# 12334zq/optical-flow-1

Hardware: AMD Instinct MI355X
Metric: Mpix*warp-iters/s, TV-L1 1920x1080 5-scale (higher is better)
Workload: dtype f64; 1 GPU; tvl1flow 1920x1080 pair (synthetic P1), nscales=5 warps=5 tau=0.25 lambda=0.15 theta=0.3 zfactor=0.5 epsilon=0.01; one pair per step per GPU; workload_name=1080p, arithmetic_mode=tolerance, pairs_per_gpu=1040, pairs_in_flight_per_gpu=64, lockstep_group=16, streams_per_gpu=4, distinct_pairs=8

## Files before the change

optical-flow-1_amd/csrc/ofx_tvl1.hip:

```cpp
#include "ofx_ops.h"
#include "ofx_device.h"
#include "ofx_loop.h"

#include <atomic>
#include <chrono>
#include <cmath>
#include <thread>
#include <type_traits>

#define TVL1_GRAD_IS_ZERO 1E-10
#define TVL1_PRESMOOTHING_SIGMA 0.8
#define STRIP_OUT 62

template <typename T> OFX_DEV double rnd_to(double x);
template <> OFX_DEV double rnd_to<double>(double x) { return x; }
template <> OFX_DEV double rnd_to<float>(double x) { return (double) (float) x; }

#ifdef OFX_NO_RFL
#define OFX_WAVE_UNIFORM(x) (x)
#else
#define OFX_WAVE_UNIFORM(x) __builtin_amdgcn_readfirstlane(x)
#endif
template <typename T> struct RowIn {
    double2 u, p1, p2, a;
// ... 753 lines not shown
    const bool idle = (strip >= strips_x) || (y0 >= ny);
    const int yend = (y0 + rows < ny) ? y0 + rows : ny;
    const int ys = y0 > N - 1 ? y0 - (N - 1) : 0;
    const int yl = (yend + N - 1 < ny - 1) ? yend + N - 1 : ny - 1;
    const int c = strip * STRIP3_OUT - STRIP3_HALO + lane;
    const int cc = c < 0 ? 0 : (c > nx - 1 ? nx - 1 : c);
    const bool lef = (c == 0), rig = (c == nx - 1);
    const bool owner = (lane >= STRIP3_HALO) && (lane < STRIP3_OUT + STRIP3_HALO) && (c < nx);
    const unsigned E2 = 2 * sizeof(T);
    const unsigned row2 = (unsigned) nx * E2;
    const unsigned off = ((unsigned) ys * nx + cc) * E2;
    const unsigned so = ((unsigned) ys * nx + (c < 0 ? 0 : c)) * E2;
    double up12 = 0.0, up22 = 0.0;
    RowIn<T> cur;
    if (!idle) {
        if (ys > 0) {
            up12 = ldw2(at(P1in, off - row2)).y;
            up22 = ldw2(at(P2in, off - row2)).y;
        }
        cur = tvl1_load_row<T>(Uin, P1in, P2in, A, R, off);
    }
    if (check) {
        double e1 = 0.0;
#pragma unroll
        for (int i = 0; i < N; i++) {
            if (k0 - i > 0) {
                const double e = loop_error_from_sum(wave_allreduce_sum(prev[i]), nx * ny, OFX_CRIT_MEAN);
                if (!(e > eps2)) return;
                if (i == 0) e1 = e;
            }
        }
        if (dev) {
            niter = (k0 > 0 && e1 <= eps2 * afac1) ? 1 : ((k0 > 0 && e1 <= eps2 * afac2) ? 2 : 3);
            if (N == 4 && niter == 3 && !(k0 > 0 && e1 <= eps2 * afac3)) niter = 4;
            if (niter > max_iter - k0) niter = max_iter - k0;
            if (scribe) dev->cursor[(launch + 1) & 1][g] = k0 + niter;
        }
    }
    if (idle) return;
    const int step = check ? 1 : 0;
    if (N == 4 && niter >= 4) {
        if constexpr (N == 4)
            tvl1_iter3_march<T, NT, STRICT, 4, N>(Uin, P1in, P2in, A, R, hu.out, h1.out, h2.out, err, slot0, step, gw, nx, ny, y0, yend,
                                                  ys, yl, lef, rig, owner, off, so, up12, up22, cur, l_t, theta, taut, ring);
    } else if (niter >= 3)
        tvl1_iter3_march<T, NT, STRICT, 3, N>(Uin, P1in, P2in, A, R, hu.out, h1.out, h2.out, err, slot0, step, gw, nx, ny, y0, yend, ys,
                                              yl, lef, rig, owner, off, so, up12, up22, cur, l_t, theta, taut);
    else if (niter == 2)
        tvl1_iter3_march<T, NT, STRICT, 2, N>(Uin, P1in, P2in, A, R, hu.out, h1.out, h2.out, err, slot0, step, gw, nx, ny, y0, yend, ys,
                                              yl, lef, rig, owner, off, so, up12, up22, cur, l_t, theta, taut);
    else
        tvl1_iter3_march<T, NT, STRICT, 1, N>(Uin, P1in, P2in, A, R, hu.out, h1.out, h2.out, err, slot0, step, gw, nx, ny, y0, yend, ys,
                                              yl, lef, rig, owner, off, so, up12, up22, cur, l_t, theta, taut);
}

template <typename T, bool NT, bool STRICT>
__global__ __launch_bounds__(256) __attribute__((amdgpu_waves_per_eu(OFX_ITER3_WAVES, OFX_ITER3_WAVES))) void k_tvl1_iter3(
    Tri<typename Pix<T>::v2> Ut, Tri<typename Pix<T>::v2> P1t, Tri<typename Pix<T>::v2> P2t,
    const typename Pix<T>::v2 *__restrict__ Ag, const T *__restrict__ Rg, double *__restrict__ errg, int k0, int check, int slot0,
    int nx, int ny, int rows, int strips_x, int strips_pad, double l_t, double theta, double taut, double eps2, unsigned incode,
    unsigned runmask, unsigned long long nit, int err_stride, OfxLoopDev *dev, int launch, double afac1, double afac2, double afac3,
    int max_iter)
{
    tvl1_unit<T, NT, STRICT, 3>(Ut, P1t, P2t, Ag, Rg, errg, k0, check, slot0, nx, ny, rows, strips_x, strips_pad, l_t, theta, taut, eps2,
                                incode, runmask, nit, err_stride, dev, launch, afac1, afac2, afac3, max_iter, nullptr);
}

template <typename T, bool NT, bool STRICT>
__global__ __launch_bounds__(256) __attribute__((amdgpu_waves_per_eu(OFX_ITER3_WAVES, OFX_ITER3_WAVES))) void k_tvl1_iter4(
    Tri<typename Pix<T>::v2> Ut, Tri<typename Pix<T>::v2> P1t, Tri<typename Pix<T>::v2> P2t,
    const typename Pix<T>::v2 *__restrict__ Ag, const T *__restrict__ Rg, double *__restrict__ errg, int k0, int check, int slot0,
    int nx, int ny, int rows, int strips_x, int strips_pad, double l_t, double theta, double taut, double eps2, unsigned incode,
    unsigned runmask, unsigned long long nit, int err_stride, OfxLoopDev *dev, int launch, double afac1, double afac2, double afac3,
    int max_iter)
{
    __shared__ Tvl1Ring rings[4];
    tvl1_unit<T, NT, STRICT, 4>(Ut, P1t, P2t, Ag, Rg, errg, k0, check, slot0, nx, ny, rows, strips_x, strips_pad, l_t, theta, taut, eps2,
                                incode, runmask, nit, err_stride, dev, launch, afac1, afac2, afac3, max_iter, &rings[threadIdx.x >> 6]);
}

#define TILE_RH 16
template <typename T, bool STRICT, int K>
__global__ __launch_bounds__(64 * TILE_RH) void k_tvl1_tile(
    Tri<typename Pix<T>::v2> Ut, Tri<typename Pix<T>::v2> P1t, Tri<typename Pix<T>::v2> P2t,
    const typename Pix<T>::v2 *__restrict__ Ag, const T *__restrict__ Rg, double *__restrict__ errg, int k0, int check, int slot0,
    int nx, int ny, int tiles_x, double l_t, double theta, double taut, double eps2, unsigned incode, unsigned runmask,
    unsigned long long nit, int err_stride)
{
    using v2 = typename Pix<T>::v2;
    static_assert(K < 16, "4 bits of `nit` per pair");
    __shared__ double2 s_p[2][TILE_RH][64];
    __shared__ double2 s_u[2][TILE_RH][64];
    const int lane = threadIdx.x & 63, w = threadIdx.x >> 6;
    const int g = blockIdx.y;
    if (!((runmask >> g) & 1u)) return;
    const int niter = (int) ((nit >> (4 * g)) & 15ull);
    const size_t npix = (size_t) nx * ny;
    const TriSel<v2> hu = pick3(Ut, incode, g, npix), h1 = pick3(P1t, incode, g, npix), h2 = pick3(P2t, incode, g, npix);
    double *__restrict__ err = errg + (size_t) g * err_stride;
    double prev[K];
#pragma unroll
    for (int i = 0; i < K; i++) prev[i] = (check && k0 - i > 0) ? loop_fetch_prev(err, k0 - i) : 0.0;

    constexpr int OW = 64 - 2 * K, OH = TILE_RH - 2 * K;
    const int tx = blockIdx.x % tiles_x, ty = blockIdx.x / tiles_x;
    const int c = tx * OW - K + lane, y = ty * OH - K + w;
    const int cc = c < 0 ? 0 : (c > nx - 1 ? nx - 1 : c), yc = y < 0 ? 0 : (y > ny - 1 ? ny - 1 : y);
    const bool inside = (c >= 0) && (c < nx) && (y >= 0) && (y < ny);
    const bool owner = inside && lane >= K && lane < 64 - K && w >= K && w < TILE_RH - K;
    const bool lef = (c == 0), rig = (c == nx - 1), top = (y == 0), bot = (y == ny - 1);
    const size_t p = (size_t) yc * nx + cc;
    double2 u = ldw2(hu.in + p), p1 = ldw2(h1.in + p), p2 = ldw2(h2.in + p);
    const double2 a = ldw2(Ag + (size_t) g * npix + p);
    const double r = ldw(Rg + (size_t) g * npix + p);
    if (check) {
#pragma unroll
        for (int i = 0; i < K; i++)
            if (k0 - i > 0 && !(loop_error_from_sum(wave_allreduce_sum(prev[i]), nx * ny, OFX_CRIT_MEAN) > eps2)) return;
    }
    double acc[K];
#pragma unroll
    for (int it = 0; it < K; it++) {
        acc[it] = 0.0;
        if (it < niter) {
            s_p[it & 1][w][lane] = make_double2(p1.y, p2.y);
            __syncthreads();
            const double2 up = s_p[it & 1][w > 0 ? w - 1 : 0][lane];
            const double l11 = wave_shift_up(p1.x), l21 = wave_shift_up(p2.x);
            const double2 un = tvl1_primal<T, STRICT>(u, a, r, p1, p2, l11, l21, up.x, up.y, lef, rig, top, bot, l_t, theta);
            if (owner) acc[it] = TVL1_TOL64<T, STRICT> ? du2_fma(un, u)
                : (un.x - u.x) * (un.x - u.x) + (un.y - u.y) * (un.y - u.y);
            s_u[it & 1][w][lane] = un;
            __syncthreads();
            const double2 dn = s_u[it & 1][w < TILE_RH - 1 ? w + 1 : w][lane];
            const double r1 = wave_shift_down(un.x), r2 = wave_shift_down(un.y);
            double2 q1, q2;
            tvl1_dual<T, STRICT>(p1, p2, un, r1, r2, dn, rig, bot, taut, q1, q2);
            u = un;
            p1 = make_double2(rnd_to<T>(q1.x), rnd_to<T>(q1.y));
            p2 = make_double2(rnd_to<T>(q2.x), rnd_to<T>(q2.y));
        }
    }
    if (owner) {
        const size_t po = (size_t) y * nx + c;
        stn2(hu.out + po, u);
        stn2(h1.out + po, p1);
        stn2(h2.out + po, p2);
    }
#pragma unroll
    for (int it = 0; it < K; it++)
        if (it < niter) loop_accumulate(err, slot0 + (check ? it : 0), acc[it], blockIdx.x * TILE_RH + w);
}

#ifndef OFX_WARP_BX
#define OFX_WARP_BX 64
#define OFX_WARP_BY 4
#endif
template <typename T>
__global__ void k_tvl1_warp(const typename Pix<T>::v2 *__restrict__ pag, const T *__restrict__ pbg, const T *__restrict__ I0g,
                            Tri<typename Pix<T>::v2> Ut,
                            typename Pix<T>::v2 *__restrict__ Ag, T *__restrict__ Rg, int nx, int ny, unsigned curcode)
{
    const int j = blockIdx.x * OFX_WARP_BX + threadIdx.x;
    const int i = blockIdx.y * OFX_WARP_BY + threadIdx.y;
    if (j >= nx || i >= ny) return;
    const int g = blockIdx.z;
    const size_t goff = (size_t) g * nx * ny;
    const typename Pix<T>::v2 *__restrict__ pa = pag + goff;
    const T *__restrict__ pb = pbg + goff;
    const T *__restrict__ I0 = I0g + goff;
    const typename Pix<T>::v2 *__restrict__ U = pick3(Ut, curcode, g, (size_t) nx * ny).in;
    typename Pix<T>::v2 *__restrict__ A = Ag + goff;
    T *__restrict__ R = Rg + goff;
    const size_t p = (size_t) i * nx + j;
    const double2 u = ldw2(U + p);
    const BicubicTaps t = bicubic_taps(j + u.x, i + u.y, nx, ny);
    double I1w = 0.0, I1wx = 0.0, I1wy = 0.0;
    if (!t.out) {
        bicubic_sample3(pa, pb, t, nx, I1w, I1wx, I1wy);
        I1wx = rnd_to<T>(I1wx);
        I1wy = rnd_to<T>(I1wy);
    }
    stn2(A + p, make_double2(I1wx, I1wy));
    stn(R + p, (I1w - I1wx * u.x - I1wy * u.y - ldw(I0 + p)));
}

#ifndef WARP_TW
#define WARP_TW 48
#define WARP_TH 16
#endif
#ifndef WARP_BY
#define WARP_BY 8
#endif
#ifndef WARP_WAVES
#define WARP_WAVES 8
#endif
#define WARP_ATTR __attribute__((amdgpu_waves_per_eu(WARP_WAVES, WARP_WAVES)))
#define WARP_NT (32 * WARP_BY)
#define WARP_NW (WARP_NT / 64)
template <typename T>
__global__ __launch_bounds__(WARP_NT) WARP_ATTR void k_tvl1_warp_lds(
    const typename Pix<T>::v2 *__restrict__ pag, const T *__restrict__ pbg, const T *__restrict__ I0g,
    Tri<typename Pix<T>::v2> Ut, typename Pix<T>::v2 *__restrict__ Ag, T *__restrict__ Rg, int nx, int ny,
    unsigned curcode)
{
    __shared__ double2 s_a[WARP_TH * WARP_TW];
    __shared__ double s_b[WARP_TH * WARP_TW];
    __shared__ int s_box[WARP_NW][4];
    const int tid = threadIdx.y * 32 + threadIdx.x, wave = tid >> 6;
    const int j = blockIdx.x * 32 + threadIdx.x;
    const int i = blockIdx.y * WARP_BY + threadIdx.y;
    const bool inside = (j < nx) && (i < ny);
    const int g = blockIdx.z;
    const size_t goff = (size_t) g * nx * ny;
    const typename Pix<T>::v2 *__restrict__ pa = pag + goff;
    const T *__restrict__ pb = pbg + goff;
    const typename Pix<T>::v2 *__restrict__ U = pick3(Ut, curcode, g, (size_t) nx * ny).in;
    const size_t p = (size_t) (inside ? i : 0) * nx + (inside ? j : 0);
    double2 u = make_double2(0.0, 0.0);
    BicubicTaps t;
    t.out = true;
    if (inside) {
        u = ldw2(U + p);
        t = bicubic_taps(j + u.x, i + u.y, nx, ny);
    }
    const bool need = inside && !t.out;
    int xlo = need ? t.col[0] : 0x7fffffff, xhi = need ? t.col[3] : -1;
    int ylo = need ? t.row[0] : 0x7fffffff, yhi = need ? t.row[3] : -1;
#pragma unroll
    for (int m = 32; m >= 1; m >>= 1) {
        xlo = min(xlo, __shfl_xor(xlo, m, 64)); xhi = max(xhi, __shfl_xor(xhi, m, 64));
        ylo = min(ylo, __shfl_xor(ylo, m, 64)); yhi = max(yhi, __shfl_xor(yhi, m, 64));
    }
    if ((tid & 63) == 0) { s_box[wave][0] = xlo; s_box[wave][1] = xhi; s_box[wave][2] = ylo; s_box[wave][3] = yhi; }
    __syncthreads();
#pragma unroll
    for (int w = 0; w < WARP_NW; w++) {
        xlo = min(xlo, s_box[w][0]); xhi = max(xhi, s_box[w][1]);
        ylo = min(ylo, s_box[w][2]); yhi = max(yhi, s_box[w][3]);
    }
    const int W = xhi - xlo + 1, H = yhi - ylo + 1;
    const bool any = (xhi >= 0);
    const bool tile = any && W <= WARP_TW && H <= WARP_TH;
    if (tile) {
        for (int k = tid; k < W * H; k += WARP_NT) {
            const int r = k / W, c = k - r * W;
            const size_t src = (size_t) (ylo + r) * nx + (xlo + c);
            s_a[r * WARP_TW + c] = ldw2(pa + src);
            s_b[r * WARP_TW + c] = ldw(pb + src);
        }
        __syncthreads();
    }
    if (!inside) return;
    double I1w = 0.0, I1wx = 0.0, I1wy = 0.0;
    if (need) {
        if (tile) {
            const int cx = t.col[0] - xlo, cy = t.row[0] - ylo;
            double c0[4], c1[4], c2[4];
#pragma unroll
            for (int k = 0; k < 4; k++) {
                const int o = cy * WARP_TW + cx + k;
                const double2 a0 = s_a[o], a1 = s_a[o + WARP_TW], a2 = s_a[o + 2 * WARP_TW], a3 = s_a[o + 3 * WARP_TW];
                const double b0 = s_b[o], b1 = s_b[o + WARP_TW], b2 = s_b[o + 2 * WARP_TW], b3 = s_b[o + 3 * WARP_TW];
                c0[k] = cubic_cell(a0.x, a1.x, a2.x, a3.x, t.fy);
                c1[k] = cubic_cell(a0.y, a1.y, a2.y, a3.y, t.fy);
                c2[k] = cubic_cell(b0, b1, b2, b3, t.fy);
            }
            I1w = cubic_cell(c0[0], c0[1], c0[2], c0[3], t.fx);
            I1wx = cubic_cell(c1[0], c1[1], c1[2], c1[3], t.fx);
            I1wy = cubic_cell(c2[0], c2[1], c2[2], c2[3], t.fx);
        } else {
            bicubic_sample3(pa, pb, t, nx, I1w, I1wx, I1wy);
        }
        I1wx = rnd_to<T>(I1wx);
        I1wy = rnd_to<T>(I1wy);
    }
    stn2(Ag + goff + p, make_double2(I1wx, I1wy));
    stn(Rg + goff + p, (I1w - I1wx * u.x - I1wy * u.y - ldw(I0g + goff + p)));
}

template <typename T>
__global__ void k_tvl1_zoom_in_g(Tri<typename Pix<T>::v2> Ut, unsigned curcode, typename Pix<T>::v2 *__restrict__ Uout, int nx,
                                 int ny, int nxx, int nyy, double fx, double fy, double scale)
{
    const int j1 = blockIdx.x * 64 + threadIdx.x;
    const int i1 = blockIdx.y * 4 + threadIdx.y;
    if (j1 >= nxx || i1 >= nyy) return;
    const int g = blockIdx.z;
    const typename Pix<T>::v2 *__restrict__ U = pick3(Ut, curcode, g, (size_t) nx * ny).in;
    const double i2 = i1 / fy, j2 = j1 / fx;
    const BicubicTaps t = bicubic_taps(j2, i2, nx, ny);
    double c1[4], c2[4];
#pragma unroll
    for (int k = 0; k < 4; k++) {
        const double2 v0 = ldw2(U + (size_t) t.row[0] * nx + t.col[k]);
        const double2 v1 = ldw2(U + (size_t) t.row[1] * nx + t.col[k]);
        const double2 v2 = ldw2(U + (size_t) t.row[2] * nx + t.col[k]);
        const double2 v3 = ldw2(U + (size_t) t.row[3] * nx + t.col[k]);
        c1[k] = cubic_cell(v0.x, v1.x, v2.x, v3.x, t.fy);
        c2[k] = cubic_cell(v0.y, v1.y, v2.y, v3.y, t.fy);
    }
    double2 r;
    r.x = cubic_cell(c1[0], c1[1], c1[2], c1[3], t.fx) * scale;
    r.y = cubic_cell(c2[0], c2[1], c2[2], c2[3], t.fx) * scale;
    stn2(Uout + (size_t) g * nxx * nyy + (size_t) i1 * nxx + j1, r);
}

template <typename T>
__global__ void k_tvl1_to_flo_g(Tri<typename Pix<T>::v2> Ut, unsigned curcode, OfxGroupPtrs out, size_t n)
{
    const size_t i = (size_t) blockIdx.x * blockDim.x + threadIdx.x;
    if (i >= n) return;
    const int g = blockIdx.y;
    const double2 v = ldw2(pick3(Ut, curcode, g, n).in + i);
    ((float2 *) out.a[g])[i] = make_float2((float) v.x, (float) v.y);
}

template <typename T> struct Tvl1Level {
    using v2 = typename Pix<T>::v2;
    using v4 = typename Pix<T>::v4;
    int nx, ny, G;
    int shared;
    T  *I0, *I1;
    v2 *pa;
    T  *pb;
    v2 *U[3], *P1[3], *P2[3], *A;
    T  *R;
    unsigned cur;
    int last_n[OFX_MAX_GROUP];
    size_t n() const { return (size_t) nx * ny; }
    unsigned curidx(int g) const { return (cur >> (2 * g)) & 3u; }
    v2 *Ucur(int g) const { return U[curidx(g)] + (size_t) g * n(); }
    v2 *P1cur(int g) const { return P1[curidx(g)] + (size_t) g * n(); }
    v2 *P2cur(int g) const { return P2[curidx(g)] + (size_t) g * n(); }
    Tri<v2> Ut() const { return Tri<v2>{U[0], U[1], U[2]}; }
    Tri<v2> P1t() const { return Tri<v2>{P1[0], P1[1], P1[2]}; }
    Tri<v2> P2t() const { return Tri<v2>{P2[0], P2[1], P2[2]}; }
};

struct Tvl1Params {
    double tau, lambda, theta, epsilon;
    int warps, verbose, max_iter;
    bool fixed;
};

template <typename T> static int tvl1_level_alloc(ofx_ctx *ctx, Tvl1Level<T> &L, int nx, int ny, int G, bool images, int shared = 0)
{
    const size_t n = (size_t) nx * ny * G;
    L.nx = nx;
    L.ny = ny;
    L.G = G;
    L.shared = shared;
    L.cur = 0;
    for (int g = 0; g < OFX_MAX_GROUP; g++) L.last_n[g] = 0;
    L.I0 = L.I1 = nullptr;
    if (images) {
        OFX_TRY(ofx_alloc(ctx, n, &L.I0));
        if (!shared) OFX_TRY(ofx_alloc(ctx, n, &L.I1));
    }
    OFX_TRY(ofx_alloc(ctx, n, &L.pa));
    OFX_TRY(ofx_alloc(ctx, n, &L.pb));
    for (int h = 0; h < 3; h++) {
        OFX_TRY(ofx_alloc(ctx, n, &L.U[h]));
        OFX_TRY(ofx_alloc(ctx, n, &L.P1[h]));
        OFX_TRY(ofx_alloc(ctx, n, &L.P2[h]));
    }
    OFX_TRY(ofx_alloc(ctx, n, &L.A));
    OFX_TRY(ofx_alloc(ctx, n, &L.R));
    return OFX_OK;
}

static int tvl1_pick_rows(const ofx_ctx *ctx, int nx, int ny, int G)
{
    if (ctx->rows_per_wave > 0) return ctx->rows_per_wave;
    const long strips = (long) ofx_cdiv(nx, STRIP_OUT) * G;
    if (strips * ofx_cdiv(ny, 4) >= 2048) return 4;
    if (strips * ofx_cdiv(ny, 2) >= 1024) return 2;
    return 1;
}

static int tvl1_pick_rows2(const ofx_ctx *ctx, int nx, int ny, int G)
{
    if (ctx->rows_per_wave2 > 0) return ctx->rows_per_wave2;
    const long strips_pad = (long) ofx_cdiv(ofx_cdiv(nx, STRIP2_OUT), 4) * 4 * G;
    const int rmax = 24;
    int best = rmax;
    long best_cost = -1;
    if (ctx->concurrency > 1) {
        static const int cand[] = {1, 2, 3, 4, 5, 6, 8, 10, 12, 14, 16, 20, 24};
        for (int r : cand) {
            const long waves = strips_pad * ofx_cdiv(ny, r);
            const long slots = ctx->rows_slots > 0 ? ctx->rows_slots : 1024;
            const long cost = ((waves + slots - 1) / slots) * (r + 5);
            if (best_cost < 0 || cost < best_cost) { best_cost = cost; best = r; }
        }
        return best;
    }
    const long slots = 1024L * OFX_ITER2_WAVES;
    for (int k = 1; k <= 4; k++) {
        for (int r = 1; r <= rmax; r++) {
            if (strips_pad * ofx_cdiv(ny, r) > k * slots) continue;
            const long cost = (long) k * (r + 5);
            if (best_cost < 0 || cost < best_cost) { best_cost = cost; best = r; }
            break;
        }
    }
    if (best < 3 && strips_pad * ofx_cdiv(ny, 3) >= 512) best = 3;
    return best;
}

static int tvl1_pick_chunk(const ofx_ctx *ctx, int nx, int ny, int G)
{
    if (ctx->chunk > 0) return ctx->chunk;
    const double est_us = fmax(5.0, (double) nx * ny * G * 120.0 / 4.0e6);
    int c = (int) (40.0 / est_us);
    return c < 4 ? 4 : (c > 50 ? 50 : c);
}

static int tvl1_pick_tile(const ofx_ctx *ctx, int nx, int ny, int G)
{
    if (!ctx->tile || !ctx->fuse2) return 0;
    const double lim = ctx->tile_max_px > 0 ? ctx->tile_max_px : 200000.0;
    if ((double) nx * ny * G > lim) return 0;
    return ctx->tile == 6 ? 6 : 4;
}

template <typename T> struct Tvl1Level;
struct Tvl1Params;
template <typename T>
static int tvl1_run_iterations_tile(ofx_ctx *ctx, Tvl1Level<T> &L, const Tvl1Params &P, LoopSpec S, int K, int *n_out,
                                    double *err_out, float *ms_out, int *alt_out);
template <typename T>
static int tvl1_run_iterations_tri(ofx_ctx *ctx, Tvl1Level<T> &L, const Tvl1Params &P, LoopSpec S, int N, int *n_out, double *err_out,
                                   float *ms_out, int *alt_out);

static int tvl1_pick_rows3(const ofx_ctx *ctx, int nx, int ny, int G, int N = 3)
{
    const int depth = 2 * N + 1;
    if (ctx->rows_per_wave3 > 0) return ctx->rows_per_wave3;
    {
        static const char *tab = getenv("OFX_ROWS3");
        for (const char *q = tab; q && *q;) {
            int lny = 0, r = 0;
            if (sscanf(q, "%d:%d", &lny, &r) == 2 && lny == ny && r > 0) return r;
            q = strchr(q, '/');
            if (q) q++;
        }
    }
    const long strips_pad = (long) ofx_cdiv(ofx_cdiv(nx, STRIP3_OUT), 4) * 4 * G;
    const int rmax = 32;
    int best = rmax;
    long best_cost = -1;
    if (ctx->concurrency > 1) {
        static const int cand[] = {2, 3, 4, 5, 6, 8, 10, 12, 14, 16, 20, 24, 28, 32, 36, 40, 48, 54, 64, 72, 80, 96};
        for (int r : cand) {
            if (r > ctx->rows3_max) break;
            const long waves = strips_pad * ofx_cdiv(ny, r);
            const long slots = ctx->rows_slots > 0 ? ctx->rows_slots : 1024;
            const long cost = ((waves + slots - 1) / slots) * (r + depth);
            if (best_cost < 0 || cost < best_cost) { best_cost = cost; best = r; }
        }
        return best;
    }
    const long slots = 1024L * OFX_ITER3_WAVES;
    for (int k = 1; k <= 4; k++) {
        for (int r = 1; r <= rmax; r++) {
            if (strips_pad * ofx_cdiv(ny, r) > k * slots) continue;
            const long cost = (long) k * (r + depth);
            if (best_cost < 0 || cost < best_cost) { best_cost = cost; best = r; }
            break;
        }
    }
    if (best < 4 && strips_pad * ofx_cdiv(ny, 4) >= 512) best = 4;
    return best;
}

#ifndef TVL1_FUSE4_AUTO_PX
#define TVL1_FUSE4_AUTO_PX 2e6
#endif
template <typename T>
static int tvl1_run_iterations(ofx_ctx *ctx, Tvl1Level<T> &L, const Tvl1Params &P, int *n_out, double *err_out,
                               float *ms_out, int *alt_out = nullptr,
                               int *unit_out = nullptr)
{
    const int nx = L.nx, ny = L.ny, G = L.G;
    if ((long long) nx * ny >= (1LL << 27)) return ofx_fail(ctx, OFX_ERR_ARG, "tvl1: image larger than 2^27 pixels");
    const double l_t = P.lambda * P.theta, taut = P.tau / P.theta, theta = P.theta;
    const bool pairs = ctx->fuse2 != 0;
    const int rows = tvl1_pick_rows(ctx, nx, ny, G);
    const int strips_x = ofx_cdiv(nx, STRIP_OUT), strips_pad = ofx_cdiv(strips_x, 4) * 4;
    const unsigned gx1 = (unsigned) (strips_pad / 4) * ofx_cdiv(ny, rows);
    const dim3 block(256);
    const int rows2 = tvl1_pick_rows2(ctx, nx, ny, G);
    const int strips2_x = ofx_cdiv(nx, STRIP2_OUT), strips2_pad = ofx_cdiv(strips2_x, 4) * 4;
    const dim3 grid2((unsigned) (strips2_pad / 4) * ofx_cdiv(ny, rows2), G);
    LoopSpec S;
    S.max_iter = P.max_iter;
    S.size = nx * ny;
    S.thr = P.epsilon * P.epsilon;
    S.crit = OFX_CRIT_MEAN;
    S.chunk = tvl1_pick_chunk(ctx, nx, ny, G);
    S.fixed = P.fixed;
    S.pairs = pairs;
    const int tileK = tvl1_pick_tile(ctx, nx, ny, G);
    if (unit_out) *unit_out = tileK ? tileK : (pairs ? 2 : 1);
    if (tileK) return tvl1_run_iterations_tile<T>(ctx, L, P, S, tileK, n_out, err_out, ms_out, alt_out);
    {
        const bool strict_mode = sizeof(T) == sizeof(double) && !ctx->relaxed_dual;
        const double px = (double) nx * ny * G;
        const bool tri = ctx->fuse3 == 1 ? px >= ctx->fuse3_min_px
                                         : (ctx->fuse3 == 2 && !strict_mode && (G >= 2 || ctx->concurrency > 1) &&
                                            px >= (ctx->fuse3_min_px > 0 ? ctx->fuse3_min_px : 5e5));
        const bool quad = ctx->fuse4 == 1 ? px >= ctx->fuse4_min_px
                                          : (ctx->fuse4 == 2 && tri && ctx->fuse3 == 2 &&
// ... 81 lines not shown
    S.afac = 0.0;
    if (ctx->chunk <= 0) S.chunk = 6 * K;
    const int err_stride = (S.max_iter + 1) * OFX_NSHARD;
    const unsigned all = (G >= 32) ? 0xFFFFFFFFu : ((1u << G) - 1u);
    unsigned b0[OFX_MAX_GROUP];
    for (int g = 0; g < G; g++) b0[g] = L.curidx(g);
    auto go = [&](int k0, int check, int slot0, double thr, unsigned incode, unsigned runmask, unsigned long long nit) -> int {
        auto kern = K == 6 ? k_tvl1_tile<T, false, 6> : k_tvl1_tile<T, false, 4>;
        if constexpr (sizeof(T) == sizeof(double)) {
            if (strict) kern = K == 6 ? k_tvl1_tile<T, true, 6> : k_tvl1_tile<T, true, 4>;
        }
        hipLaunchKernelGGL(kern, grid, block, 0, ctx->stream, L.Ut(), L.P1t(), L.P2t(), L.A, (const T *) L.R, ctx->d_err, k0, check,
                           slot0, nx, ny, tiles_x, l_t, theta, taut, thr, incode, runmask, nit, err_stride);
        OFX_LAUNCH_CHECK(ctx);
        return OFX_OK;
    };
    auto launch = [&](int k, int cnt, double thr) -> int {
        unsigned incode = 0;
        unsigned long long nit = 0;
        for (int g = 0; g < G; g++) {
            incode |= ((b0[g] + (unsigned) (k / K)) % 3u) << (2 * g);
            nit |= (unsigned long long) cnt << (4 * g);
        }
        return go(k, 1, k, thr, incode, all, nit);
    };
    auto redo = [&](const int *k_of) -> int {
        unsigned incode = 0, runmask = 0;
        unsigned long long nit = 0;
        for (int g = 0; g < G; g++) {
            if (k_of[g] < 0) continue;
            const int n = k_of[g] + 1, j = (n - 1) / K;
            runmask |= 1u << g;
            incode |= ((b0[g] + (unsigned) j) % 3u) << (2 * g);
            nit |= (unsigned long long) (n - j * K) << (4 * g);
        }
        return go(0, 0, S.max_iter, -1.0, incode, runmask, nit);
    };
    int took_alt[OFX_MAX_GROUP];
    OFX_TRY(ofx_run_loop_group(ctx, S, G, launch, redo, n_out, err_out, ms_out, 0u, took_alt));
    unsigned cur = 0;
    for (int g = 0; g < G; g++) {
        const unsigned units = (unsigned) ((n_out[g] + K - 1) / K);
        cur |= ((b0[g] + units) % 3u) << (2 * g);
        L.last_n[g] = n_out[g];
        if (alt_out) alt_out[g] = 0;
    }
    L.cur = cur;
    return OFX_OK;
}

template <typename T>
static int tvl1_run_iterations_tri(ofx_ctx *ctx, Tvl1Level<T> &L, const Tvl1Params &P, LoopSpec S, int N, int *n_out, double *err_out,
                                   float *ms_out, int *alt_out)
{
    const int nx = L.nx, ny = L.ny, G = L.G;
    const double l_t = P.lambda * P.theta, taut = P.tau / P.theta, theta = P.theta;
    const bool strict = sizeof(T) == sizeof(double) && !ctx->relaxed_dual;
    const int rows = tvl1_pick_rows3(ctx, nx, ny, G, N);
    const int strips_x = ofx_cdiv(nx, STRIP3_OUT), strips_pad = ofx_cdiv(strips_x, 4) * 4;
    const dim3 grid((unsigned) (strips_pad / 4) * ofx_cdiv(ny, rows), G), block(256);
    const bool nt_stores = ctx->nt_stores ? ctx->nt_stores == 1 : (double) nx * ny * G * 15.0 * sizeof(T) > 300e6;
    S.pairs = false;
    S.fuse = N;
    S.afac = 0.0;
    const int err_stride = (S.max_iter + 1) * OFX_NSHARD;
    const unsigned all = (G >= 32) ? 0xFFFFFFFFu : ((1u << G) - 1u);
    unsigned b0[OFX_MAX_GROUP];
    for (int g = 0; g < G; g++) b0[g] = L.curidx(g);
    const bool cursor = ctx->fuse3_cursor != 0 && !S.fixed;
    const double afac2 = ctx->fuse3_afac2 > 0 ? ctx->fuse3_afac2 : 1.5, afac1 = ctx->fuse3_afac1 > 0 ? ctx->fuse3_afac1 : 1.2;
    const double afac3 = ctx->fuse4_afac3 > 0 ? ctx->fuse4_afac3 : afac2;
    auto go = [&](int k0, int check, int slot0, double thr, unsigned incode, unsigned runmask, unsigned long long nit, OfxLoopDev *dev,
                  int launch) -> int {
        auto kern = nt_stores ? k_tvl1_iter3<T, true, false> : k_tvl1_iter3<T, false, false>;
        if (N == 4) kern = nt_stores ? k_tvl1_iter4<T, true, false> : k_tvl1_iter4<T, false, false>;
        if constexpr (sizeof(T) == sizeof(double)) {
            if (strict) kern = nt_stores ? k_tvl1_iter3<T, true, true> : k_tvl1_iter3<T, false, true>;
            if (strict && N == 4) kern = nt_stores ? k_tvl1_iter4<T, true, true> : k_tvl1_iter4<T, false, true>;
        }
        hipLaunchKernelGGL(kern, grid, block, 0, ctx->stream, L.Ut(), L.P1t(), L.P2t(), L.A, (const T *) L.R, ctx->d_err, k0, check,
                           slot0, nx, ny, rows, strips_x, strips_pad, l_t, theta, taut, thr, incode, runmask, nit, err_stride, dev, launch,
                           afac1, afac2, afac3, S.max_iter);
        OFX_LAUNCH_CHECK(ctx);
        return OFX_OK;
    };
    auto code_of_unit = [&](unsigned unit) -> unsigned {
        unsigned c = 0;
        for (int g = 0; g < G; g++) c |= ((b0[g] + unit) % 3u) << (2 * g);
        return c;
    };
    int unit_of[OFX_MAX_GROUP];
    int inside[OFX_MAX_GROUP];
    if (cursor) {
        auto launch = [&](int Lidx, double thr) -> int {
            return go(0, 1, 0, thr, code_of_unit((unsigned) Lidx), all, 0ull, reinterpret_cast<OfxLoopDev *>(ctx->d_state), Lidx);
        };
        auto redo = [&](const int *n_of, const int *k0_of, const int *u_of) -> int {
            unsigned incode = 0, runmask = 0;
            unsigned long long nit = 0;
            for (int g = 0; g < G; g++) {
                if (n_of[g] < 0) continue;
                runmask |= 1u << g;
                incode |= ((b0[g] + (unsigned) u_of[g]) % 3u) << (2 * g);
                nit |= (unsigned long long) (n_of[g] - k0_of[g]) << (4 * g);
            }
            return go(0, 0, S.max_iter, -1.0, incode, runmask, nit, nullptr, 0);
        };
        const int upc = (S.chunk + N - 1) / N < 1 ? 1 : (S.chunk + N - 1) / N;
        OFX_TRY(ofx_run_loop_cursor(ctx, S, G, upc, N, launch, redo, n_out, err_out, unit_of, inside, ms_out));
    } else {
        auto launch = [&](int k, int cnt, double thr) -> int {
            unsigned long long nit = 0;
            for (int g = 0; g < G; g++) nit |= (unsigned long long) cnt << (4 * g);
            return go(k, 1, k, thr, code_of_unit((unsigned) (k / N)), all, nit, nullptr, 0);
        };
        auto redo = [&](const int *k_of) -> int {
            unsigned incode = 0, runmask = 0;
            unsigned long long nit = 0;
            for (int g = 0; g < G; g++) {
                if (k_of[g] < 0) continue;
                const int n = k_of[g] + 1, j = (n - 1) / N;
                runmask |= 1u << g;
                incode |= ((b0[g] + (unsigned) j) % 3u) << (2 * g);
                nit |= (unsigned long long) (n - j * N) << (4 * g);
            }
            return go(0, 0, S.max_iter, -1.0, incode, runmask, nit, nullptr, 0);
        };
        int took_alt[OFX_MAX_GROUP];
        OFX_TRY(ofx_run_loop_group(ctx, S, G, launch, redo, n_out, err_out, ms_out, 0u, took_alt));
        for (int g = 0; g < G; g++) {
            unit_of[g] = n_out[g] > 0 ? (n_out[g] - 1) / N : -1;
            inside[g] = (n_out[g] % N != 0 && n_out[g] != S.max_iter) ? 1 : 0;
        }
    }
    unsigned cur = 0;
    for (int g = 0; g < G; g++) {
        const unsigned units = (unsigned) (unit_of[g] + 1);
        cur |= ((b0[g] + units) % 3u) << (2 * g);
        L.last_n[g] = n_out[g];
        if (alt_out) alt_out[g] = inside[g] ? 1 : 0;
    }
    L.cur = cur;
    return OFX_OK;
}

template <typename T>
static int tvl1_single_scale_dev(ofx_ctx *ctx, Tvl1Level<T> &L, const Tvl1Params &P, int scale, ofx_stats *stats)
{
    const int nx = L.nx, ny = L.ny, G = L.G;
    const size_t n = L.n();
    const dim3 g2(ofx_cdiv(nx, OFX_WARP_BX), ofx_cdiv(ny, OFX_WARP_BY), G), b2(OFX_WARP_BX, OFX_WARP_BY);
    if (nx < 2 || ny < 2) return ofx_fail(ctx, OFX_ERR_ARG, "tvl1: level %dx%d too small", nx, ny);

    if (!L.shared) {
        OFX_TRY(op_grad_pack<T>(ctx, L.I1, L.pa, L.pb, nx, ny, G));
    } else {
        const size_t half = n * L.shared;
        OFX_TRY(op_grad_pack<T>(ctx, L.I0 + half, L.pa, L.pb, nx, ny, L.shared));
        OFX_TRY(op_grad_pack<T>(ctx, L.I0, L.pa + half, L.pb + half, nx, ny, L.shared));
    }
    for (int h = 0; h < 3; h++) {
        bool used = false;
        for (int g = 0; g < G; g++) used = used || (L.curidx(g) == (unsigned) h);
        if (!used) continue;
        OFX_TRY(op_fill2<T>(ctx, L.P1[h], n * G));
        OFX_TRY(op_fill2<T>(ctx, L.P2[h], n * G));
    }
    for (int g = 0; g < G; g++) L.last_n[g] = 0;

    for (int w = 0; w < P.warps; w++) {
        if (ctx->warp_lds)
            hipLaunchKernelGGL(k_tvl1_warp_lds<T>, dim3(ofx_cdiv(nx, 32), ofx_cdiv(ny, WARP_BY), G), dim3(32, WARP_BY), 0, ctx->stream, L.pa,
                               (const T *) L.pb, (const T *) L.I0, L.Ut(), L.A, L.R, nx, ny, L.cur);
        else
            hipLaunchKernelGGL(k_tvl1_warp<T>, g2, b2, 0, ctx->stream, L.pa, (const T *) L.pb, (const T *) L.I0, L.Ut(),
                               L.A, L.R, nx, ny, L.cur);
        OFX_LAUNCH_CHECK(ctx);
        int it[OFX_MAX_GROUP];
        double error[OFX_MAX_GROUP];
        float ms = 0.f;
        int odd[OFX_MAX_GROUP], unit = 0;
        OFX_TRY(tvl1_run_iterations<T>(ctx, L, P, it, error, ctx->profile ? &ms : nullptr, odd, &unit));
        if (P.verbose && G == 1) fprintf(stderr, "Warping: %d, Iterations: %d, Error: %f\n", w, it[0], error[0]);
        for (int g = 0; g < G; g++) {
            ofx_stats &S = stats[g];
            S.odd_stops += odd[g] != 0;
            S.odd_stops_stored += odd[g] == 2;
            if (scale < OFX_MAX_SCALES) {
                S.fused[scale] = unit;
                if (w < OFX_MAX_SOLVES) { S.iters[scale][w] = it[g]; S.error[scale][w] = error[g]; }
                S.iter_ms[scale] += ms;
                S.iter_launches[scale] += it[g];
            }
            S.work_pix_iters += (double) it[g] * nx * ny;
        }
    }
    return OFX_OK;
}

static void stats_begin(ofx_stats *st, int nscales, int nsolves)
{
    memset(st, 0, sizeof(*st));
    st->nscales = nscales;
    st->nsolves = nsolves;
}

template <typename T>
static int tvl1_multiscale_dev(ofx_ctx *ctx, int G, const T *const *dI0, const T *const *dI1, int nxx, int nyy,
                               const Tvl1Params &P, int nscales, double zfactor, std::vector<Tvl1Level<T>> &lv,
                               ofx_stats *stats, int kind = -1, size_t pitch = 0,
                               int shared = 0,
                               const void *const *init = nullptr)
{
    const int Gp = shared ? shared : G;
    if (shared && G != 2 * shared) return ofx_fail(ctx, OFX_ERR_ARG, "tvl1: %d slots for %d bidirectional pairs", G, shared);
    if (P.warps < 1) return ofx_fail(ctx, OFX_ERR_ARG, "tvl1: warps=%d", P.warps);
    if (G < 1 || G > OFX_MAX_GROUP) return ofx_fail(ctx, OFX_ERR_ARG, "tvl1: group of %d pairs", G);

    std::vector<int> nxs, nys;
    OFX_TRY(op_pyramid_sizes(ctx, nxx, nyy, nscales, zfactor, nxs, nys));
    for (int g = 0; g < G; g++) {
        stats_begin(&stats[g], nscales, P.warps);
        for (int s = 0; s < nscales && s < OFX_MAX_SCALES; s++) { stats[g].nx[s] = nxs[s]; stats[g].ny[s] = nys[s]; }
    }
    lv.resize(nscales);
    for (int s = 0; s < nscales; s++) OFX_TRY(tvl1_level_alloc<T>(ctx, lv[s], nxs[s], nys[s], G, true, shared));
    {
        T *tmpA, *tmpB;
        double *scr;
        OFX_TRY(ofx_alloc(ctx, (size_t) 2 * Gp * nxx * nyy, &tmpA));
        OFX_TRY(ofx_alloc(ctx, (size_t) 2 * Gp * nxx * nyy, &tmpB));
        OFX_TRY(ofx_alloc(ctx, (size_t) Gp * op_pyramid_scratch_doubles(), &scr));
        std::vector<T *> lA(nscales), lB(nscales);
        for (int s = 0; s < nscales; s++) { lA[s] = lv[s].I0; lB[s] = shared ? lv[s].I0 + (size_t) shared * lv[s].n() : lv[s].I1; }
        OFX_TRY(op_build_pyramid_group<T>(ctx, Gp, (const void *const *) dI0, (const void *const *) dI1, nscales, zfactor,
                                          TVL1_PRESMOOTHING_SIGMA, nxs.data(), nys.data(), lA.data(), lB.data(), tmpA, tmpB, scr, kind,
                                          pitch));
    }
    Tvl1Level<T> &C = lv[nscales - 1];
    if (!init) {
        OFX_TRY(op_fill2<T>(ctx, C.U[0], C.n() * G));
    } else {
        void *dst[OFX_MAX_GROUP];
        for (int g = 0; g < G; g++) dst[g] = C.U[0] + (size_t) g * C.n();
        OFX_TRY(op_flow_pyramid<typename Pix<T>::v2>(ctx, G, init, nscales, zfactor, nxs.data(), nys.data(), dst));
    }

    for (int s = nscales - 1; s >= 0; s--) {
        if (P.verbose && G == 1) fprintf(stderr, "Scale %d: %dx%d\n", s, lv[s].nx, lv[s].ny);
        OFX_TRY(tvl1_single_scale_dev<T>(ctx, lv[s], P, s, stats));
        if (!s) break;
        lv[s - 1].cur = 0;
        {
            const int nxf = lv[s - 1].nx, nyf = lv[s - 1].ny;
            hipLaunchKernelGGL(k_tvl1_zoom_in_g<T>, dim3(ofx_cdiv(nxf, 64), ofx_cdiv(nyf, 4), G), dim3(64, 4), 0, ctx->stream,
                               lv[s].Ut(), lv[s].cur, lv[s - 1].U[0], lv[s].nx, lv[s].ny, nxf, nyf, (double) nxf / lv[s].nx,
                               (double) nyf / lv[s].ny, 1.0 / zfactor);
            OFX_LAUNCH_CHECK(ctx);
        }
    }
    return OFX_OK;
}

static Tvl1Params make_params(const ofx_ctx *ctx, double tau, double lambda, double theta, int warps,
                               double epsilon, int verbose)
{
    Tvl1Params P;
    P.tau = tau; P.lambda = lambda; P.theta = theta; P.epsilon = epsilon;
    P.warps = warps; P.verbose = verbose;
    P.max_iter = OFX_TVL1_MAX_ITERATIONS;
    P.fixed = ctx->fixed_work != 0;
    return P;
}

template <typename T>
static int upload_image(ofx_ctx *ctx, const double *h, size_t n, T **out)
{
    double *stage;
    OFX_TRY(ofx_alloc(ctx, n, &stage));
    OFX_TRY(ofx_alloc(ctx, n, out));
    OFX_HIP(ctx, hipMemcpyAsync(stage, h, n * sizeof(double), hipMemcpyHostToDevice, ctx->stream));
    return op_convert_in<T>(ctx, stage, *out, n);
}

template <typename T>
static int tvl1_multiscale_host(ofx_ctx *ctx, const double *I0, const double *I1, double *u1, double *u2, int nx,
                                int ny, const Tvl1Params &P, int nscales, double zfactor)
{
    const size_t n = (size_t) nx * ny;
    T *dI0, *dI1;
    OFX_TRY(upload_image<T>(ctx, I0, n, &dI0));
    OFX_TRY(upload_image<T>(ctx, I1, n, &dI1));
    std::vector<Tvl1Level<T>> lv;
    const T *a = dI0, *b = dI1;
    OFX_TRY(tvl1_multiscale_dev<T>(ctx, 1, &a, &b, nx, ny, P, nscales, zfactor, lv, &ctx->stats));
    double *d1, *d2;
    OFX_TRY(ofx_alloc(ctx, n, &d1));
    OFX_TRY(ofx_alloc(ctx, n, &d2));
    OFX_TRY(op_deinterleave2<T>(ctx, lv[0].Ucur(0), d1, d2, n));
    OFX_HIP(ctx, hipMemcpyAsync(u1, d1, n * sizeof(double), hipMemcpyDeviceToHost, ctx->stream));
    OFX_HIP(ctx, hipMemcpyAsync(u2, d2, n * sizeof(double), hipMemcpyDeviceToHost, ctx->stream));
    OFX_HIP(ctx, hipStreamSynchronize(ctx->stream));
    return OFX_OK;
}

extern "C" int ofx_tvl1_multiscale(ofx_ctx *ctx, const double *I0, const double *I1, double *u1, double *u2, int nx,
                                   int ny, double tau, double lambda, double theta, int nscales, double zfactor,
                                   int warps, double epsilon, int verbose)
{
    OFX_ENTER(ctx);
    if (!I0 || !I1 || !u1 || !u2) return ofx_fail(ctx, OFX_ERR_ARG, "tvl1: NULL pointer");
    const double t0 = ofx_now_ms();
    const Tvl1Params P = make_params(ctx, tau, lambda, theta, warps, epsilon, verbose);
    int s = ctx->precision == OFX_F64
                ? tvl1_multiscale_host<double>(ctx, I0, I1, u1, u2, nx, ny, P, nscales, zfactor)
                : tvl1_multiscale_host<float>(ctx, I0, I1, u1, u2, nx, ny, P, nscales, zfactor);
    ctx->stats.total_ms = ofx_now_ms() - t0;
    return s;
}

bool ofx_ptr_is_local(const ofx_ctx *ctx, const void *p)
{
    hipPointerAttribute_t a;
    if (hipPointerGetAttributes(&a, p) != hipSuccess) {
        (void) hipGetLastError();
        return false;
    }
    return a.type == hipMemoryTypeDevice && a.device == ctx->device;
// ... 572 lines not shown
```

Measured before the change: 88880 Mpix*warp-iters/s.

## Fuse gradient computation into warp kernel, drop precomputed gradient buffers

Removes the per-scale grad_pack pass and the pa/pb buffers. The warp kernels now read the raw second image and compute central-difference gradients on the fly, staging a haloed image tile in LDS and deriving gradients there, with a register-sliding path for the non-tile fallback. This cuts a full-image kernel pass and the memory traffic of packed gradients per scale, at the cost of extra ALU and LDS work in each of the five warp launches. Clamped boundary gradients may differ from the original grad_pack if it used one-sided differences at the borders.

```diff
diff --git a/optical-flow-1_amd/csrc/ofx_tvl1.hip b/optical-flow-1_amd/csrc/ofx_tvl1.hip
--- a/optical-flow-1_amd/csrc/ofx_tvl1.hip
+++ b/optical-flow-1_amd/csrc/ofx_tvl1.hip
@@ -929,13 +929,57 @@
         if (it < niter) loop_accumulate(err, slot0 + (check ? it : 0), acc[it], blockIdx.x * TILE_RH + w);
 }
 
+template <typename T>
+OFX_DEV void bicubic_sample3_i1(const T *__restrict__ I1, const BicubicTaps &t, int nx, int ny, double &o0, double &o1, double &o2)
+{
+    const int r0 = t.row[0], q0 = t.col[0];
+    auto at = [=](int r, int c) {
+        const int rr = min(max(r0 + r, 0), ny - 1), cc = min(max(q0 + c, 0), nx - 1);
+        return ldw(reinterpret_cast<const T *>(reinterpret_cast<const char *>(I1) +
+                                               ((unsigned) rr * (unsigned) nx + (unsigned) cc) * (unsigned) sizeof(T)));
+    };
+    double c0[4], c1[4], c2[4], l[4], m[6], n[4];
+#pragma unroll
+    for (int r = 0; r < 4; r++) l[r] = at(r, -1);
+#pragma unroll
+    for (int r = 0; r < 6; r++) m[r] = at(r - 1, 0);
+#pragma unroll
+    for (int k = 0; k < 4; k++) {
+        double gx[4], gy[4];
+#pragma unroll
+        for (int r = 0; r < 4; r++) {
+            n[r] = at(r, k + 1);
+            gx[r] = rnd_to<T>(0.5 * (n[r] - l[r]));
+            gy[r] = rnd_to<T>(0.5 * (m[r + 2] - m[r]));
+        }
+        c0[k] = cubic_cell(m[1], m[2], m[3], m[4], t.fy);
+        c1[k] = cubic_cell(gx[0], gx[1], gx[2], gx[3], t.fy);
+        c2[k] = cubic_cell(gy[0], gy[1], gy[2], gy[3], t.fy);
+        if (k < 3) {
+#pragma unroll
+            for (int r = 0; r < 4; r++) { l[r] = m[r + 1]; m[r + 1] = n[r]; }
+            m[0] = at(-1, k + 1);
+            m[5] = at(4, k + 1);
+        }
+    }
+    o0 = cubic_cell(c0[0], c0[1], c0[2], c0[3], t.fx);
+    o1 = cubic_cell(c1[0], c1[1], c1[2], c1[3], t.fx);
+    o2 = cubic_cell(c2[0], c2[1], c2[2], c2[3], t.fx);
+}
+
+template <typename T> OFX_DEV const T *tvl1_second_image(const T *base, int g, int shift, size_t npix)
+{
+    const int G = (int) gridDim.z;
+    const int pl = g + shift < G ? g + shift : g + shift - G;
+    return base + (size_t) pl * npix;
+}
+
 #ifndef OFX_WARP_BX
 #define OFX_WARP_BX 64
 #define OFX_WARP_BY 4
 #endif
 template <typename T>
-__global__ void k_tvl1_warp(const typename Pix<T>::v2 *__restrict__ pag, const T *__restrict__ pbg, const T *__restrict__ I0g,
-                            Tri<typename Pix<T>::v2> Ut,
+__global__ void k_tvl1_warp(const T *__restrict__ I1g, int shift, const T *__restrict__ I0g, Tri<typename Pix<T>::v2> Ut,
                             typename Pix<T>::v2 *__restrict__ Ag, T *__restrict__ Rg, int nx, int ny, unsigned curcode)
 {
     const int j = blockIdx.x * OFX_WARP_BX + threadIdx.x;
@@ -943,8 +987,7 @@
     if (j >= nx || i >= ny) return;
     const int g = blockIdx.z;
     const size_t goff = (size_t) g * nx * ny;
-    const typename Pix<T>::v2 *__restrict__ pa = pag + goff;
-    const T *__restrict__ pb = pbg + goff;
+    const T *__restrict__ I1 = tvl1_second_image(I1g, g, shift, (size_t) nx * ny);
     const T *__restrict__ I0 = I0g + goff;
     const typename Pix<T>::v2 *__restrict__ U = pick3(Ut, curcode, g, (size_t) nx * ny).in;
     typename Pix<T>::v2 *__restrict__ A = Ag + goff;
@@ -954,7 +997,7 @@
     const BicubicTaps t = bicubic_taps(j + u.x, i + u.y, nx, ny);
     double I1w = 0.0, I1wx = 0.0, I1wy = 0.0;
     if (!t.out) {
-        bicubic_sample3(pa, pb, t, nx, I1w, I1wx, I1wy);
+        bicubic_sample3_i1<T>(I1, t, nx, ny, I1w, I1wx, I1wy);
         I1wx = rnd_to<T>(I1wx);
         I1wy = rnd_to<T>(I1wy);
     }
@@ -975,14 +1018,14 @@
 #define WARP_ATTR __attribute__((amdgpu_waves_per_eu(WARP_WAVES, WARP_WAVES)))
 #define WARP_NT (32 * WARP_BY)
 #define WARP_NW (WARP_NT / 64)
+#define WARP_LW (WARP_TW + 2)
 template <typename T>
 __global__ __launch_bounds__(WARP_NT) WARP_ATTR void k_tvl1_warp_lds(
-    const typename Pix<T>::v2 *__restrict__ pag, const T *__restrict__ pbg, const T *__restrict__ I0g,
-    Tri<typename Pix<T>::v2> Ut, typename Pix<T>::v2 *__restrict__ Ag, T *__restrict__ Rg, int nx, int ny,
-    unsigned curcode)
-{
-    __shared__ double2 s_a[WARP_TH * WARP_TW];
-    __shared__ double s_b[WARP_TH * WARP_TW];
+    const T *__restrict__ I1g, int shift, const T *__restrict__ I0g, Tri<typename Pix<T>::v2> Ut,
+    typename Pix<T>::v2 *__restrict__ Ag, T *__restrict__ Rg, int nx, int ny, unsigned curcode)
+{
+    __shared__ double s_i[(WARP_TH + 2) * WARP_LW];
+    __shared__ double2 s_g[WARP_TH * WARP_TW];
     __shared__ int s_box[WARP_NW][4];
     const int tid = threadIdx.y * 32 + threadIdx.x, wave = tid >> 6;
     const int j = blockIdx.x * 32 + threadIdx.x;
@@ -990,8 +1033,7 @@
     const bool inside = (j < nx) && (i < ny);
     const int g = blockIdx.z;
     const size_t goff = (size_t) g * nx * ny;
-    const typename Pix<T>::v2 *__restrict__ pa = pag + goff;
-    const T *__restrict__ pb = pbg + goff;
+    const T *__restrict__ I1 = tvl1_second_image(I1g, g, shift, (size_t) nx * ny);
     const typename Pix<T>::v2 *__restrict__ U = pick3(Ut, curcode, g, (size_t) nx * ny).in;
     const size_t p = (size_t) (inside ? i : 0) * nx + (inside ? j : 0);
     double2 u = make_double2(0.0, 0.0);
@@ -1020,11 +1062,17 @@
     const bool any = (xhi >= 0);
     const bool tile = any && W <= WARP_TW && H <= WARP_TH;
     if (tile) {
+        const int W2 = W + 2;
+        for (int k = tid; k < W2 * (H + 2); k += WARP_NT) {
+            const int r = k / W2, c = k - r * W2;
+            const int rr = min(max(ylo - 1 + r, 0), ny - 1), cc = min(max(xlo - 1 + c, 0), nx - 1);
+            s_i[r * WARP_LW + c] = ldw(I1 + (size_t) rr * nx + cc);
+        }
+        __syncthreads();
         for (int k = tid; k < W * H; k += WARP_NT) {
             const int r = k / W, c = k - r * W;
-            const size_t src = (size_t) (ylo + r) * nx + (xlo + c);
-            s_a[r * WARP_TW + c] = ldw2(pa + src);
-            s_b[r * WARP_TW + c] = ldw(pb + src);
+            const double *q = s_i + (r + 1) * WARP_LW + (c + 1);
+            s_g[r * WARP_TW + c] = make_double2(rnd_to<T>(0.5 * (q[1] - q[-1])), rnd_to<T>(0.5 * (q[WARP_LW] - q[-WARP_LW])));
         }
         __syncthreads();
     }
@@ -1036,18 +1084,18 @@
             double c0[4], c1[4], c2[4];
 #pragma unroll
             for (int k = 0; k < 4; k++) {
-                const int o = cy * WARP_TW + cx + k;
-                const double2 a0 = s_a[o], a1 = s_a[o + WARP_TW], a2 = s_a[o + 2 * WARP_TW], a3 = s_a[o + 3 * WARP_TW];
-                const double b0 = s_b[o], b1 = s_b[o + WARP_TW], b2 = s_b[o + 2 * WARP_TW], b3 = s_b[o + 3 * WARP_TW];
-                c0[k] = cubic_cell(a0.x, a1.x, a2.x, a3.x, t.fy);
-                c1[k] = cubic_cell(a0.y, a1.y, a2.y, a3.y, t.fy);
-                c2[k] = cubic_cell(b0, b1, b2, b3, t.fy);
+                const int oi = (cy + 1) * WARP_LW + cx + 1 + k, og = cy * WARP_TW + cx + k;
+                const double i0 = s_i[oi], i1 = s_i[oi + WARP_LW], i2 = s_i[oi + 2 * WARP_LW], i3 = s_i[oi + 3 * WARP_LW];
+                const double2 g0 = s_g[og], g1 = s_g[og + WARP_TW], g2 = s_g[og + 2 * WARP_TW], g3 = s_g[og + 3 * WARP_TW];
+                c0[k] = cubic_cell(i0, i1, i2, i3, t.fy);
+                c1[k] = cubic_cell(g0.x, g1.x, g2.x, g3.x, t.fy);
+                c2[k] = cubic_cell(g0.y, g1.y, g2.y, g3.y, t.fy);
             }
             I1w = cubic_cell(c0[0], c0[1], c0[2], c0[3], t.fx);
             I1wx = cubic_cell(c1[0], c1[1], c1[2], c1[3], t.fx);
             I1wy = cubic_cell(c2[0], c2[1], c2[2], c2[3], t.fx);
         } else {
-            bicubic_sample3(pa, pb, t, nx, I1w, I1wx, I1wy);
+            bicubic_sample3_i1<T>(I1, t, nx, ny, I1w, I1wx, I1wy);
         }
         I1wx = rnd_to<T>(I1wx);
         I1wy = rnd_to<T>(I1wy);
@@ -1099,8 +1147,6 @@
     int nx, ny, G;
     int shared;
     T  *I0, *I1;
-    v2 *pa;
-    T  *pb;
     v2 *U[3], *P1[3], *P2[3], *A;
     T  *R;
     unsigned cur;
@@ -1135,8 +1181,6 @@
         OFX_TRY(ofx_alloc(ctx, n, &L.I0));
         if (!shared) OFX_TRY(ofx_alloc(ctx, n, &L.I1));
     }
-    OFX_TRY(ofx_alloc(ctx, n, &L.pa));
-    OFX_TRY(ofx_alloc(ctx, n, &L.pb));
     for (int h = 0; h < 3; h++) {
         OFX_TRY(ofx_alloc(ctx, n, &L.U[h]));
         OFX_TRY(ofx_alloc(ctx, n, &L.P1[h]));
@@ -1524,13 +1568,7 @@
     const dim3 g2(ofx_cdiv(nx, OFX_WARP_BX), ofx_cdiv(ny, OFX_WARP_BY), G), b2(OFX_WARP_BX, OFX_WARP_BY);
     if (nx < 2 || ny < 2) return ofx_fail(ctx, OFX_ERR_ARG, "tvl1: level %dx%d too small", nx, ny);
 
-    if (!L.shared) {
-        OFX_TRY(op_grad_pack<T>(ctx, L.I1, L.pa, L.pb, nx, ny, G));
-    } else {
-        const size_t half = n * L.shared;
-        OFX_TRY(op_grad_pack<T>(ctx, L.I0 + half, L.pa, L.pb, nx, ny, L.shared));
-        OFX_TRY(op_grad_pack<T>(ctx, L.I0, L.pa + half, L.pb + half, nx, ny, L.shared));
-    }
+    const T *second = L.shared ? L.I0 : L.I1;
     for (int h = 0; h < 3; h++) {
         bool used = false;
         for (int g = 0; g < G; g++) used = used || (L.curidx(g) == (unsigned) h);
@@ -1542,10 +1580,10 @@
 
     for (int w = 0; w < P.warps; w++) {
         if (ctx->warp_lds)
-            hipLaunchKernelGGL(k_tvl1_warp_lds<T>, dim3(ofx_cdiv(nx, 32), ofx_cdiv(ny, WARP_BY), G), dim3(32, WARP_BY), 0, ctx->stream, L.pa,
-                               (const T *) L.pb, (const T *) L.I0, L.Ut(), L.A, L.R, nx, ny, L.cur);
+            hipLaunchKernelGGL(k_tvl1_warp_lds<T>, dim3(ofx_cdiv(nx, 32), ofx_cdiv(ny, WARP_BY), G), dim3(32, WARP_BY), 0, ctx->stream, second,
+                               L.shared, (const T *) L.I0, L.Ut(), L.A, L.R, nx, ny, L.cur);
         else
-            hipLaunchKernelGGL(k_tvl1_warp<T>, g2, b2, 0, ctx->stream, L.pa, (const T *) L.pb, (const T *) L.I0, L.Ut(),
+            hipLaunchKernelGGL(k_tvl1_warp<T>, g2, b2, 0, ctx->stream, second, L.shared, (const T *) L.I0, L.Ut(),
                                L.A, L.R, nx, ny, L.cur);
         OFX_LAUNCH_CHECK(ctx);
         int it[OFX_MAX_GROUP];
```

Measured after the change: 89320 Mpix*warp-iters/s (median of 5 runs). About the same (+0.5%).
